# chaiyujin/sdfa-2019

Hardware: AMD Instinct MI355X
Metric: animation frames/s/node (10 s@16 kHz clips); max|Δdgrad| vs CPU ref (higher is better)
Workload: dtype f32

## Files before the change

include/sdfa_hip.h:

```cpp
#ifndef SDFA_HIP_H
#define SDFA_HIP_H

#include <stdint.h>

#ifdef __cplusplus
extern "C" {
#endif

#define SDFA_ABI_VERSION 5

#define SDFA_OK            0
#define SDFA_EINVAL       -1
#define SDFA_ESHORTCLIP   -2
#define SDFA_EHIP         -3
#define SDFA_ESTATE       -4
#define SDFA_ENOSPACE     -5

#define SDFA_HEAD_DGRAD    0
#define SDFA_HEAD_OFFSETS  1

#define SDFA_FEAT_FRAMES   64
#define SDFA_FEAT_MELS    128
#define SDFA_FEAT_CH        3
#define SDFA_Z_DIM        512
// ... 27 lines not shown
int         sdfa_model_finalize(sdfa_model *m, void *stream);
int         sdfa_model_head(const sdfa_model *m);
int64_t     sdfa_model_out_dim(const sdfa_model *m);
int64_t     sdfa_model_coef_dim(const sdfa_model *m);

#define SDFA_PREC_FP32 0
#define SDFA_PREC_BF16_ATTENTION 1
#define SDFA_PREC_BF16X3 2
#define SDFA_PREC_BF16 3
#define SDFA_PREC_BF16X3_ATTENTION 4
#define SDFA_PREC_BF16X6 5
int         sdfa_model_set_precision(sdfa_model *m, int mode);
int         sdfa_model_precision(const sdfa_model *m);

int         sdfa_model_autotune(sdfa_model *m, int64_t n_frames, void *d_workspace, int64_t workspace_bytes, void *stream);

int         sdfa_model_set_reserved_cus(sdfa_model *m, int k);

int64_t sdfa_workspace_bytes(const sdfa_model *m, int64_t max_frames);

#define SDFA_WS_STATUS_BYTES 256
#define SDFA_WS_STATUS_WORDS 4
#define SDFA_WS_TIME_LSTM_REPAIRS 0
int     sdfa_workspace_init(void *d_workspace, int64_t workspace_bytes, void *stream);
int     sdfa_workspace_status_async(const void *d_workspace, uint32_t *h_status, void *stream);
int64_t sdfa_workspace_status(const void *d_workspace, int word, void *stream);

int sdfa_encoder_forward(const sdfa_model *m, const float *d_audio_feat, int64_t n_frames,
                         float *d_z, float *d_align, void *d_workspace, int64_t workspace_bytes,
                         void *stream);

int sdfa_encoder_forward_shared(const sdfa_model *m, const float *d_audio_feat, int64_t n_frames,
                                const int32_t *d_frame_clip, const int64_t *d_frame_start, int hop,
                                float *d_z, float *d_align, void *d_workspace, int64_t workspace_bytes,
                                void *stream);

int sdfa_regress_forward(const sdfa_model *m, const float *d_z, const int64_t *d_speaker_id,
                         int64_t n_frames, float *d_coef, float *d_out, void *d_workspace,
                         int64_t workspace_bytes, void *stream);

int sdfa_regress_forward_multi(const sdfa_model *m, const float *d_z, const int64_t *d_speaker_id, int64_t n_frames,
                               float *d_coef, float *const *h_d_outs, int n_outs, void *d_workspace,
                               int64_t workspace_bytes, void *stream);

int sdfa_expand_coef(const sdfa_model *m, const float *d_coef, int64_t n_frames, float *d_out, void *d_workspace,
                     int64_t workspace_bytes, void *stream);
// ... 54 lines not shown
```

sdfa-2019_amd/csrc/api_core.cpp:

```cpp
#include "../../include/sdfa_stream.h"
#include "host.h"

#include <climits>
#include <cstdio>
#include <cstring>
#include <string>

static thread_local std::string g_err;

int sdfa_failv(int code, const char *fmt, va_list ap) {
    char buf[512];
    vsnprintf(buf, sizeof buf, fmt, ap);
    g_err = buf;
    return code;
}

int sdfa_fail(int code, const char *fmt, ...) {
    va_list ap;
    va_start(ap, fmt);
    sdfa_failv(code, fmt, ap);
    va_end(ap);
    return code;
}

thread_local int g_sdfa_mel_fft_radix4 = 0;
thread_local int g_sdfa_gather_plain_order = 0;
thread_local int g_sdfa_frontend_two_kernel = 0;
thread_local int g_sdfa_frontend_stream_block = 0;
thread_local int g_sdfa_frontend_stream_slots = 0;
thread_local int g_sdfa_frontend_stream_spin_max = 0;
thread_local int g_sdfa_frontend_stream_phases = 0;
thread_local int g_sdfa_frontend_t_major = 0;
extern thread_local int g_sdfa_gemm_variant;
thread_local int g_sdfa_freq_lstm_shape = 0;
thread_local int g_sdfa_pca_lds = 0;
thread_local int g_sdfa_pca_fp32 = 0;
thread_local int g_sdfa_conv_fp32 = 0;
thread_local int g_sdfa_time_lstm_split = 0;
thread_local int g_sdfa_time_lstm_fuse_x = 0;
thread_local int g_sdfa_time_lstm_handoff = 0;
thread_local int g_sdfa_time_lstm_timeout_us = 0;
thread_local int g_sdfa_share_gx0_off = 0;
thread_local int g_sdfa_encoder_dedup_off = 0;
thread_local int g_sdfa_share_hash_bits = 0;
thread_local int g_sdfa_freq_proj_tail = 0;
thread_local int g_sdfa_attn_unfused = 0;

extern "C" {

int sdfa_abi_version(void) { return SDFA_ABI_VERSION; }
int sdfa_stream_abi_version(void) { return SDFA_STREAM_ABI_VERSION; }
const char *sdfa_last_error(void) { return g_err.c_str(); }

int sdfa_debug_set_option(const char *name, int value) {
    struct Option { const char *name; int *var; int lo = INT_MIN, hi = INT_MAX; const char *accepts = nullptr; };
    thread_local const Option options[] = {
        {"attn_unfused", &g_sdfa_attn_unfused},
        {"share_gx0_off", &g_sdfa_share_gx0_off},
        {"encoder_dedup_off", &g_sdfa_encoder_dedup_off},
        {"share_hash_bits", &g_sdfa_share_hash_bits, 0, 32, "0 (the whole hash) or 1..32 low bits"},
        {"freq_proj_tail", &g_sdfa_freq_proj_tail, 0, 2, "0 (rule), 1 (never) or 2 (always)"},
        {"frontend_two_kernel", &g_sdfa_frontend_two_kernel},
        {"frontend_stream_phases", &g_sdfa_frontend_stream_phases},
        {"frontend_stream_spin_max", &g_sdfa_frontend_stream_spin_max, 0, INT_MAX, "0 (default) or a positive poll count"},
        {"frontend_stream_block", &g_sdfa_frontend_stream_block, 0, 256, "0 (default) or 1..256 frames"},
        {"frontend_stream_slots", &g_sdfa_frontend_stream_slots, 0, 256, "0 (default) or 1..256 workgroups per block"},
        {"gather_plain_order", &g_sdfa_gather_plain_order},
        {"mel_fft_radix4", &g_sdfa_mel_fft_radix4},
        {"frontend_t_major", &g_sdfa_frontend_t_major},
        {"time_lstm_timeout_us", &g_sdfa_time_lstm_timeout_us},
        {"time_lstm_handoff", &g_sdfa_time_lstm_handoff},
        {"time_lstm_split", &g_sdfa_time_lstm_split},
        {"time_lstm_fuse_x", &g_sdfa_time_lstm_fuse_x, 0, 3, "0 (rule), 1 (never), 2 or 3 (always, 32- / 64-frame tiles)"},
        {"gemm_variant", &g_sdfa_gemm_variant},
        {"freq_lstm_shape", &g_sdfa_freq_lstm_shape},
        {"pca_lds", &g_sdfa_pca_lds},
        {"conv_fp32", &g_sdfa_conv_fp32},
        {"pca_fp32", &g_sdfa_pca_fp32},
    };
    for (const Option &o : options)
        if (name && !strcmp(name, o.name)) {
            if (value < o.lo || value > o.hi) return sdfa_fail(SDFA_EINVAL, "%s: %s", o.name, o.accepts);
            *o.var = value;
            return SDFA_OK;
// ... 6 lines not shown
```

sdfa-2019_amd/csrc/api_forward.cpp:

```cpp
#include "common.h"
#include "host.h"
#include "kernels.h"
#include "model.h"

#include <algorithm>

extern thread_local int g_sdfa_gemm_variant, g_sdfa_freq_lstm_shape, g_sdfa_pca_lds, g_sdfa_pca_fp32, g_sdfa_conv_fp32, g_sdfa_share_gx0_off, g_sdfa_attn_unfused, g_sdfa_encoder_dedup_off,
    g_sdfa_freq_proj_tail, g_sdfa_share_hash_bits;

namespace {

constexpr int64_t CT_WORDS = 2048, CT_FLAGS = 16, ST_WORDS = SDFA_WS_STATUS_BYTES / 4;

struct Ws {
    int64_t P1, X3, HF, Z, GX, H0, H1, KP, QC, QP, ZK, SH, ZU, total;
    int64_t TRUNK, A0, A1, COEF;
    int64_t CT_FREQ, CT_PCA, CT_FLAG;
};

Ws layout(int64_t Nc, bool keep) {
    const int64_t Mc = 64 * Nc;
    Ws w{};
    int64_t o = 0;
    auto take = [&](int64_t n) { int64_t r = o; o += round_up(n, 64); return r; };
    take(ST_WORDS);
    if (keep) {
        w.P1 = take(2048 * Mc); w.X3 = take(2048 * Mc); w.HF = take((int64_t)HF_SLAB_ROWS * 4 * Mc); w.Z = take(256 * Mc);
        w.GX = take(2048 * Mc); w.H0 = take(512 * Mc); w.H1 = take(512 * Mc); w.KP = take(128 * Mc);
    } else {
        const int64_t A = take(2048 * Mc);
        const int64_t B = take(2048 * Mc);
// ... 124 lines not shown
    if (((uintptr_t)d_workspace | (uintptr_t)d_audio_feat | (uintptr_t)d_z | (uintptr_t)d_H | (uintptr_t)d_X1) & 15) return sdfa_fail(SDFA_EINVAL, "encoder_forward: pointers must be 16-byte aligned");
    if ((uintptr_t)d_align & 3) return sdfa_fail(SDFA_EINVAL, "encoder_forward: d_align must be 4-byte aligned");
    const int64_t cap = capacity(workspace_bytes, m->keep);
    if (cap < 128) return sdfa_fail(SDFA_ENOSPACE, "encoder_forward: workspace of %lld bytes holds no 128-frame chunk", (long long)workspace_bytes);
    hipStream_t s = (hipStream_t)stream;
    Prof pf{m, s};
    float *ws = (float *)d_workspace;
    for (int64_t f0 = 0; f0 < n_frames; f0 += cap) {
        const int64_t N = std::min(cap, n_frames - f0);
        const int64_t Nc = round_up(N, 128), Mc = 64 * Nc;
        const Ws w = layout(Nc, m->keep);
        ConvArgs ca{};
        ca.audio_feat = d_audio_feat + f0 * (64 * 128 * 3); ca.N = N; ca.Nc = Nc; ca.Mc = Mc;
        ca.w1 = m->w1; ca.b1 = m->b1; ca.s1 = m->s1; ca.t1 = m->t1; ca.P1 = ws + w.P1;
        ca.w2 = m->w2; ca.b2 = m->b2; ca.s2 = m->s2; ca.t2 = m->t2;
        ca.w3 = m->w3; ca.b3 = m->b3; ca.s3 = m->s3; ca.t3 = m->t3; ca.X3 = ws + w.X3;
        const bool table = d_frame_clip != nullptr;
        const bool share = table || (!m->keep && !g_sdfa_encoder_dedup_off);
        const int64_t *d_ulimit = nullptr;
        int32_t *col_to_u = nullptr;
        bool split_tail = false;
        int64_t fat_grid = 0;
        const int64_t *d_qfull = nullptr;
        if (share) {
            ShareArgs sa{};
            sa.N = N; sa.Nc = Nc; sa.Mc = Mc;
            sdfa_share_carve(sa, reinterpret_cast<int32_t *>(ws + w.SH));
            split_tail = !m->keep && stage_terms(m, STAGE_BODY) == 0 && g_sdfa_gemm_variant == 0 && Mc / 256 >= 512 && g_sdfa_freq_proj_tail != 1;
            if (split_tail) {
                fat_grid = sdfa_fat_grid(256, Mc, sdfa_cu_count(), m->reserved_cus.load());
                sa.fat_grid = (int)fat_grid; sa.tail_mode = g_sdfa_freq_proj_tail;
            }
            pf.begin("share_map");
            if (table) {
                sa.frame_clip = d_frame_clip + f0; sa.frame_start = d_frame_start + f0; sa.hop = hop;
                sa.t_lo = 6; sa.t_hi = 58;
                HIP_TRY(sdfa_launch_share_map(sa, s));
            } else {
                sa.feat = ca.audio_feat;
                sa.hash = reinterpret_cast<uint64_t *>(ws + w.HF);
                sa.group_slots = sdfa_share_group_slots(N);
                sa.group_key = sa.hash + Mc; sa.group_first = reinterpret_cast<uint32_t *>(sa.group_key + sa.group_slots);
                sa.hash_bits = g_sdfa_share_hash_bits;
                HIP_TRY(sdfa_launch_share_map_content(sa, s));
            }
            pf.end();
            d_ulimit = sa.counts + 1; d_qfull = sa.counts + 2; col_to_u = sa.col_to_u;
            ca.col_src = sa.col_src; ca.col_limit = d_ulimit;
        }
        const int conv_terms = g_sdfa_conv_fp32 ? 0 : stage_terms(m, STAGE_BODY);
        if (m->keep && conv_terms) {
            pf.begin("conv1"); HIP_TRY(sdfa_launch_conv1(ca, s)); pf.end();
            ca.wb = m->cv_wb; ca.terms = conv_terms;
            pf.begin("conv23"); HIP_TRY(sdfa_launch_conv123(ca, s)); pf.end();
        } else if (m->keep) {
            pf.begin("conv1"); HIP_TRY(sdfa_launch_conv1(ca, s)); pf.end();
            pf.begin("conv23"); HIP_TRY(sdfa_launch_conv23(ca, s)); pf.end();
        } else {
            ca.wb = m->cv_wb; ca.terms = conv_terms;
            pf.begin("conv23"); HIP_TRY(sdfa_launch_conv123(ca, s)); pf.end();
        }

        const int fl_terms = stage_terms(m, STAGE_BODY);
        FreqLstmArgs fa{ws + w.X3, m->fl_w, m->fl_b, ws + w.HF, Mc, d_ulimit, m->fl_wb, fl_terms, reinterpret_cast<int *>(ws + w.CT_FREQ),
                        g_sdfa_freq_lstm_shape ? g_sdfa_freq_lstm_shape : (fl_terms ? 0 : m->freq_shape.load()), m->reserved_cus.load()};
        pf.begin("freq_lstm"); HIP_TRY(sdfa_launch_freq_lstm(fa, s)); pf.end();

        GemmArgs g = sdfa_gemm_k4(m->fp_w, 256, ws + w.HF, Mc, ws + w.Z, Mc, 8192);
        g.bias = m->fp_b; g.q_tile_major = 1; g.q_slab_rows = HF_SLAB_ROWS;
        g.terms = stage_terms(m, STAGE_BODY);
        g.reserve_cus = m->reserved_cus.load();
        if (share) { g.D = ws + w.ZU; g.q_limit = split_tail ? d_qfull : d_ulimit; }
        pf.begin("freq_proj");
        HIP_TRY(sdfa_launch_gemm(g, s));
        if (split_tail) {
            GemmTailArgs gt{m->fp_w, ws + w.HF, m->fp_b, ws + w.ZU, Mc, HF_SLAB_ROWS, d_qfull, d_ulimit, (int)fat_grid - 1};
            HIP_TRY(sdfa_launch_gemm_tail(gt, s));
        }
        pf.end();
        const bool share_gx0 = share && !m->keep && stage_terms(m, STAGE_BODY) == 0 && !g_sdfa_share_gx0_off;
        if (share && !share_gx0) {
            pf.begin("share_expand"); HIP_TRY(sdfa_launch_expand_cols(ws + w.ZU, col_to_u, ws + w.Z, 64, Mc, s)); pf.end();
        }

        const float *xin = share_gx0 ? ws + w.ZU : ws + w.Z;
        float *hout[2] = {ws + w.H0, ws + w.H1};
        const char *gxn[2] = {"gx0", "gx1"}, *lsn[2] = {"lstm0", "lstm1"};
        for (int l = 0; l < 2; ++l) {
            const bool mapped = share_gx0 && l == 0;
            float *gx = mapped ? ws + w.HF : ws + w.GX;
            GemmArgs gi = sdfa_gemm_k4(m->gx_w[l], 2048, xin, Mc, gx, Mc, l == 0 ? 256 : 512);
            gi.terms = stage_terms(m, STAGE_BODY);
            gi.reserve_cus = m->reserved_cus.load();
            if (mapped) gi.q_limit = d_ulimit;
            TimeLstmArgs ta{gx, m->tl_w[l], hout[l], Nc, Mc, m->tl_wb[l], stage_terms(m, STAGE_BODY),
                            reinterpret_cast<unsigned *>(ws + w.CT_FLAG), CT_WORDS - CT_FLAGS, m->tl_w16[l],
                            reinterpret_cast<unsigned *>(ws), m->reserved_cus.load(), mapped ? col_to_u : nullptr};
            if (l == 1 && !m->keep) { ta.X = xin; ta.Wxh = m->tl_wxh1; }
            pf.begin(gxn[l]);
            if (!sdfa_time_lstm_fuses_x(ta)) HIP_TRY(sdfa_launch_gemm(gi, s));
            pf.end();
            pf.begin(lsn[l]); HIP_TRY(sdfa_launch_time_lstm(ta, s)); pf.end();
            xin = hout[l];
            if (d_X1) break;
        }
        if (d_X1) {
            HIP_TRY(sdfa_launch_tap(ws + w.H0, 3, N, Nc, d_X1 + f0 * (64 * 512), s));
            continue;
        }
        const int at_terms = stage_terms(m, STAGE_ATTENTION);
        const bool key_fused = g_sdfa_attn_unfused != 1;
        pf.begin("attn_proj");
        GemmArgs gk = sdfa_gemm_k4(m->kp_w, 128, ws + w.H1, Mc, ws + w.KP, Mc, 512);
        gk.terms = at_terms;
        if (!key_fused) HIP_TRY(sdfa_launch_gemm(gk, s));
        GemmArgs gc = sdfa_gemm_k4(m->qc_w, 512, ws + w.H1 + 31 * Nc * 4, Mc, ws + w.QC, Nc, 1536);
        gc.seg_k = 512; gc.seg_col = Nc; gc.terms = at_terms;
        HIP_TRY(sdfa_launch_gemm(gc, s));
        GemmArgs gq = sdfa_gemm_k4(m->qp_w, 128, ws + w.QC, Nc, ws + w.QP, Nc, 512);
        gq.terms = at_terms;
        HIP_TRY(sdfa_launch_gemm(gq, s));
        const bool tail_fused = key_fused && (at_terms == 0 || at_terms == 6) && g_sdfa_attn_unfused != 2 && sdfa_attn_fuses_tail(Nc, m->reserved_cus.load());
        if (key_fused) {
// ... 253 lines not shown
```

sdfa-2019_amd/csrc/gemm.hip:

```cpp
#include "common.h"
#include "kernels.h"

extern thread_local int g_sdfa_gemm_variant;

namespace {

constexpr int TP = 128, TQ = 128, KQ = 8;

template <int OUT_MODE, int ACT, bool BIAS_P, bool BIAS_Q, bool COND>
__device__ __forceinline__ void store_tile(const GemmArgs &a, const f32x16 &acc, int64_t p_tile, int64_t q, int h) {
    float bq = 0.f;
    if (BIAS_Q) bq = (q < a.Qreal) ? a.bias[q] : 0.f;
    int spk = 0;
    if (COND) { spk = (int)a.cond_idx[q < a.Qreal ? q : 0]; spk = spk < 0 ? 0 : (spk > 7 ? 7 : spk); }
#pragma unroll
    for (int g = 0; g < 4; ++g) {
        const int64_t p = p_tile + 8 * g + 4 * h;
        float v[4] = {acc[4 * g + 0], acc[4 * g + 1], acc[4 * g + 2], acc[4 * g + 3]};
        if (BIAS_P) {
            float4 b = ld4(a.bias + p);
            v[0] += b.x; v[1] += b.y; v[2] += b.z; v[3] += b.w;
        }
        if (COND) {
            float4 c = ld4(a.cond_w + (p / 4 * 8 + spk) * 4);
// ... 846 lines not shown
            __builtin_amdgcn_sched_barrier(0);                                                                   \
        }                                                                                                        \
        if (fetching) FAT_DMA_NEXT()                                                                             \
        mfma_block<4, 4>(acc, fa1, fb1);                                                                         \
        mfma_block<4, 4>(acc, fa2, fb2);                                                                         \
        __builtin_amdgcn_sched_barrier(0);                                                                       \
         \
        __builtin_amdgcn_s_waitcnt(0x0070);                                                                      \
        __syncthreads();                                      \
        {               \
            const float4 *sp = SP((BUF) ^ 1), *sq = SQ((BUF) ^ 1);                                               \
            FAT_READ(sp, sq, 0, fa0, fb0)                                                                        \
            FAT_READ(sp, sq, 1, fa1, fb1)                                                                        \
            FAT_READ(sp, sq, 2, fa2, fb2)                                                                        \
            FAT_READ(sp, sq, 3, FREE_A, FREE_B)                                                                  \
            mfma_block<4, 4>(acc, LAST_A, LAST_B);                                                               \
            _Pragma("unroll") for (int m = 0; m < 8; ++m) {                                                      \
                __builtin_amdgcn_sched_group_barrier(0x100, 4, 0);                                               \
                __builtin_amdgcn_sched_group_barrier(0x008, 8, 0);                                               \
            }                                                                                                    \
        }                                                                                                        \
        __builtin_amdgcn_sched_barrier(0);                                                                       \
    }
    for (;;) {
        for (int st = 0; st < nstage; st += 2) {
            FAT_STAGE(0, fa3, fb3, fa4, fb4)
            FAT_STAGE(1, fa4, fb4, fa3, fb3)
        }
        {
            const int64_t p0 = (int64_t)t.tp * BT, q0 = (int64_t)t.tq * BT;
            char *dbase = reinterpret_cast<char *>(a.D) + (((p0 >> 2) + wp * 32) * a.ldd + q0 + wq * 128) * 16;
            const unsigned dlane = (unsigned)((h * a.ldd + l31) * 16);
#pragma unroll
            for (int i = 0; i < 4; ++i) {
                float4 b[4];
                if (BIAS_P) {
#pragma unroll
                    for (int g = 0; g < 4; ++g) b[g] = ld4(a.bias + p0 + wp * 128 + i * 32 + 8 * g + 4 * h);
                }
#pragma unroll
                for (int j = 0; j < 4; ++j) {
#pragma unroll
                    for (int g = 0; g < 4; ++g) {
                        float v[4] = {acc[i][j][4 * g + 0], acc[i][j][4 * g + 1], acc[i][j][4 * g + 2], acc[i][j][4 * g + 3]};
                        if (BIAS_P) { v[0] += b[g].x; v[1] += b[g].y; v[2] += b[g].z; v[3] += b[g].w; }
#pragma unroll
                        for (int e = 0; e < 4; ++e) {
                            if (ACT == ACT_LRELU) v[e] = lrelu02(v[e]);
                            if (ACT == ACT_TANH) v[e] = tanhf_acc(v[e]);
                        }
                        *reinterpret_cast<float4 *>(dbase + ((int64_t)(i * 8 + 2 * g) * a.ldd + j * 32) * 16 + dlane) = make_float4(v[0], v[1], v[2], v[3]);
                    }
#pragma unroll
                    for (int r = 0; r < 16; ++r) acc[i][j][r] = 0.f;
                }
            }
        }
        advance(t);
        if (!live(t)) break;
    }
#undef FAT_STAGE
#undef FAT_Q
#undef FAT_DMA_ROWS
#undef FAT_DMA_NEXT
#undef FAT_READ
}

template <int OUT_MODE, int ACT, bool BIAS_P, bool BIAS_Q, bool COND>
hipError_t launch_fat(const GemmArgs &a, hipStream_t s) {
    const size_t lds = 2 * 2 * KQ * 256 * sizeof(float4);
    hipError_t e = hipFuncSetAttribute(reinterpret_cast<const void *>(gemm_fat_kernel<OUT_MODE, ACT, BIAS_P, BIAS_Q, COND>),
                                       hipFuncAttributeMaxDynamicSharedMemorySize, (int)lds);
    if (e != hipSuccess) return e;
    const int64_t cus = sdfa_cu_count();
    const int64_t ntiles = (a.Ppad / 256) * (a.Qpad / 256);
    const int64_t wgs = std::max<int64_t>(1, cus - a.reserve_cus);
    hipLaunchKernelGGL((gemm_fat_kernel<OUT_MODE, ACT, BIAS_P, BIAS_Q, COND>), dim3((unsigned)std::min(ntiles, wgs)), dim3(256), lds, s, a);
    return hipGetLastError();
}

}

thread_local int g_sdfa_gemm_variant = 0;

template <int OUT_MODE, int ACT, bool BIAS_P, bool BIAS_Q, bool COND>
hipError_t launch_any(const GemmArgs &a, hipStream_t s) {
    const int variant = (g_sdfa_gemm_variant == 2 || g_sdfa_gemm_variant == 6 || g_sdfa_gemm_variant == 10 || g_sdfa_gemm_variant == 11) ? 0 : g_sdfa_gemm_variant;
    const bool big_fills_half = variant == 12 || (a.Ppad / 256) * (a.Qpad / 256) * 2 >= sdfa_cu_count();
    if (a.terms == 6)
// ... 1 lines not shown
                                                                                                           : launch_bf16x6<OUT_MODE, ACT, BIAS_P, BIAS_Q, COND>(a, s);
    if (a.terms) {
        const bool big = a.Ppad % 256 == 0 && a.Qpad % 256 == 0 && variant != 7 && big_fills_half;
        if (a.terms == 1) return big ? launch_bf16_big<OUT_MODE, ACT, BIAS_P, BIAS_Q, COND, 1>(a, s) : launch_bf16<OUT_MODE, ACT, BIAS_P, BIAS_Q, COND, 1>(a, s);
        return big ? launch_bf16_big<OUT_MODE, ACT, BIAS_P, BIAS_Q, COND, 3>(a, s) : launch_bf16<OUT_MODE, ACT, BIAS_P, BIAS_Q, COND, 3>(a, s);
    }
    if (variant == 4 && !a.q_tile_major) return launch_bf16<OUT_MODE, ACT, BIAS_P, BIAS_Q, COND, 3>(a, s);
    {
        const bool fits = a.Ppad % 256 == 0 && a.Qpad % 256 == 0 && a.seg_k == a.K && a.K % 64 == 0 && OUT_MODE == OUT_K4 && !BIAS_Q && !COND &&
                          a.Pstore == a.Ppad && a.ldd * 16 * 2 < (int64_t)1 << 32 &&
                          (int64_t)(a.K / 4) * a.ldp * 16 < 0x7fffffff && (int64_t)(a.K / 4) * (a.q_tile_major ? 128 : a.ldq) * 16 < 0x7fffffff;
        const int64_t ntiles = (a.Ppad / 256) * (a.Qpad / 256);
        if constexpr (OUT_MODE == OUT_K4 && !BIAS_Q && !COND) {
            if (fits && (variant == 8 || (variant == 0 && ntiles >= 512)))
                return launch_fat<OUT_MODE, ACT, BIAS_P, BIAS_Q, COND>(a, s);
        }
    }
    const bool big_fills = (a.Ppad / 256) * (a.Qpad / 256) >= 256;
    if ((variant == 5 || (a.q_tile_major && ((variant == 0 && big_fills) || variant == 9))) && a.Ppad % 256 == 0 && a.Qpad % 256 == 0)
        return launch_big<OUT_MODE, ACT, BIAS_P, BIAS_Q, COND>(a, s);
    return launch<OUT_MODE, ACT, BIAS_P, BIAS_Q, COND>(a, s);
}

hipError_t sdfa_launch_gemm(const GemmArgs &a, hipStream_t s) {
    if (a.K % 32 || a.seg_k % 32 || a.Ppad % TP || a.Qpad % TQ || a.K % a.seg_k) return hipErrorInvalidValue;
    const bool bp = a.bias && !a.bias_on_q, bq = a.bias && a.bias_on_q, cond = a.cond_w != nullptr;
    if (a.out_mode == OUT_ROW) {
        if (bq && a.act == ACT_NONE && !cond) return launch_any<OUT_ROW, ACT_NONE, false, true, false>(a, s);
        return hipErrorInvalidValue;
    }
    if (bq) return hipErrorInvalidValue;
    if (cond) {
        if (a.act == ACT_LRELU && bp) return launch_any<OUT_K4, ACT_LRELU, true, false, true>(a, s);
        return hipErrorInvalidValue;
    }
    if (a.act == ACT_NONE) return bp ? launch_any<OUT_K4, ACT_NONE, true, false, false>(a, s)
                                     : launch_any<OUT_K4, ACT_NONE, false, false, false>(a, s);
    if (a.act == ACT_TANH && bp) return launch_any<OUT_K4, ACT_TANH, true, false, false>(a, s);
    if (a.act == ACT_LRELU && bp) return launch_any<OUT_K4, ACT_LRELU, true, false, false>(a, s);
    return hipErrorInvalidValue;
}
```

sdfa-2019_amd/csrc/kernels.h:

```cpp
#pragma once
#include <hip/hip_runtime.h>
#include <stdint.h>

enum { ACT_NONE = 0, ACT_LRELU = 1, ACT_TANH = 2 };

constexpr int HF_SLAB_ROWS = 2048;
enum { OUT_K4 = 0, OUT_ROW = 1 };
constexpr int SDFA_MAX_DESTS = 8;

struct GemmArgs {
    const float *P;
    const float *Q;
    float *D;
    const float *bias;
    const float *cond_w;
    const int64_t *cond_idx;
    int64_t ldp, ldq, ldd;
    int64_t Ppad, Qpad;
    int64_t Pstore;
    int64_t Qreal;
    int K;
    int seg_k;
    int64_t seg_col;
    int act, out_mode, bias_on_q;
    int terms;
    int q_tile_major;
    int q_slab_rows;
    const int64_t *q_limit;
    int col_group, col_stride, col_off;
    float *D_extra[SDFA_MAX_DESTS - 1];
    int n_extra;
    int reserve_cus;
};
hipError_t sdfa_launch_gemm(const GemmArgs &a, hipStream_t s);
inline GemmArgs sdfa_gemm_k4(const float *P, int64_t rows, const float *Q, int64_t ldq, float *D, int64_t cols, int K) {
    GemmArgs g{};
    g.P = P; g.Q = Q; g.D = D;
    g.ldp = rows; g.Ppad = rows; g.Pstore = rows;
    g.ldq = ldq; g.ldd = cols; g.Qpad = cols; g.Qreal = cols;
    g.K = K; g.seg_k = K; g.act = ACT_NONE; g.out_mode = OUT_K4;
    return g;
}

struct PcaArgs {
    const float *coef;
    const float *basis_s, *basis_r;
    const float *mean_s, *mean_r;
    float *out;
    int64_t N, Nc, out_dim, ld_s, ld_r, cols_s, cols_r;
    float *out_extra[SDFA_MAX_DESTS - 1];
    int n_extra;
    int reserve_cus;
    const void *basis_b;
    int terms;
};
hipError_t sdfa_launch_pca_dgrad(const PcaArgs &a, hipStream_t s);
hipError_t sdfa_launch_pca_dgrad_res(const PcaArgs &a, int *queue, hipStream_t s);

struct FrontendConsts {
    const float *hamm;
    const float2 *twiddle;
    const int *mel_bin0;
    const float *mel_w8;
    int win, hop, sliding, nbins_used, nnz;
};
// ... 106 lines not shown
hipError_t sdfa_launch_k4_to_rows(const float *src, int64_t ld, int64_t N, int F, int f0, int nf, float *dst,
                                  int64_t dst_ld, hipStream_t s);
hipError_t sdfa_launch_tap(const float *src, int what, int64_t N, int64_t Nc, float *dst, hipStream_t s);

struct ShareArgs {
    const int32_t *frame_clip;
    const int64_t *frame_start;
    int hop;
    int t_lo, t_hi;
    int frame_major;
    int64_t N, Nc, Mc;
    int32_t *prev, *shift;
    int32_t *owner, *flag, *uid;
    int32_t *tile_sum;
    int32_t *col_src;
    int32_t *col_to_u;
    int64_t *counts;
    const float *feat;
    uint64_t *hash;
    uint64_t *group_key;
    uint32_t *group_first;
    int64_t group_slots;
    int hash_bits;
    int fat_grid;
    int tail_mode;
};
inline int64_t sdfa_share_table_words(int64_t Nc) { return 16 + 2 * Nc + 5 * (64 * Nc) + (64 * Nc) / 1024 + 1; }
inline int64_t sdfa_share_group_slots(int64_t N) { int64_t s = 1024; while (s < 2 * 64 * N) s <<= 1; return s; }
inline void sdfa_share_carve(ShareArgs &a, int32_t *base) {
    a.counts = reinterpret_cast<int64_t *>(base);
    a.prev = base + 16; a.shift = a.prev + a.Nc;
    a.owner = a.shift + a.Nc; a.flag = a.owner + a.Mc; a.uid = a.flag + a.Mc;
    a.col_src = a.uid + a.Mc; a.col_to_u = a.col_src + a.Mc; a.tile_sum = a.col_to_u + a.Mc;
}
hipError_t sdfa_launch_share_map(const ShareArgs &a, hipStream_t s);
hipError_t sdfa_launch_share_map_content(const ShareArgs &a, hipStream_t s);
hipError_t sdfa_launch_share_prev(const ShareArgs &a, hipStream_t s);
hipError_t sdfa_launch_expand_cols(const float *Zu, const int32_t *col_to_u, float *Z, int nquads, int64_t Mc, hipStream_t s);

struct GemmTailArgs {
    const float *P, *Q, *bias;
    float *D;
    int64_t ldd;
    int q_slab_rows;
    const int64_t *q_lo, *q_hi;
    int max_tiles;
// ... 75 lines not shown
```

sdfa-2019_amd/csrc/share.hip:

```cpp
#include "common.h"
#include "kernels.h"

namespace {


__global__ void share_prev_kernel(ShareArgs a) {
    const int64_t n = (int64_t)blockIdx.x * blockDim.x + threadIdx.x;
    if (n >= a.Nc) return;
    int prev = -1, shift = 0;
    if (n < a.N) {
        const int clip = a.frame_clip[n];
        const int64_t s = a.frame_start[n];
        for (int back = 1; back <= 64 && n - back >= 0; ++back) {
            const int64_t q = n - back;
            if (a.frame_clip[q] != clip) break;
            const int64_t diff = s - a.frame_start[q];
            if (diff <= 0) break;
            if (diff > (int64_t)(a.t_hi - a.t_lo) * a.hop) break;
            if (diff % a.hop == 0) { prev = (int)q; shift = (int)(diff / a.hop); break; }
        }
    }
    a.prev[n] = prev;
    a.shift[n] = shift;
}
// ... 118 lines not shown
}

__global__ __launch_bounds__(1024) void share_scan_tiles_kernel(ShareArgs a) {
    __shared__ int part[1024];
    const int64_t i = (int64_t)blockIdx.x * 1024 + threadIdx.x;
    const int f = i < a.Mc ? a.flag[i] : 0;
    const int inc = block_inclusive_scan_1024(f, part);
    if (i < a.Mc) a.uid[i] = inc - f;
    if (threadIdx.x == 1023) a.tile_sum[blockIdx.x] = inc;
}

constexpr int TAIL_NUM = 3, TAIL_DEN = 4;
__global__ __launch_bounds__(1024) void share_scan_sums_kernel(ShareArgs a, int ntiles) {
    __shared__ int part[1024];
    int carry = 0;
    for (int base = 0; base < ntiles; base += 1024) {
        const int t = base + threadIdx.x;
        const int v = t < ntiles ? a.tile_sum[t] : 0;
        const int inc = block_inclusive_scan_1024(v, part);
        if (t < ntiles) a.tile_sum[t] = carry + inc - v;
        carry += part[1023];
        __syncthreads();
    }
    if (threadIdx.x == 0) {
        const int64_t mu = carry, pad = (mu + 255) / 256 * 256;
        a.counts[0] = mu;
        a.counts[1] = pad;
        int64_t q_full = pad;
        if (a.fat_grid > 0 && a.tail_mode != 1) {
            const int64_t T = pad / 256, G = a.fat_grid, r = T % G;
            if (a.tail_mode == 2 || r * TAIL_DEN <= G * TAIL_NUM) q_full = (T - r) * 256;
        }
        a.counts[2] = q_full;
    }
}

__global__ __launch_bounds__(1024) void share_scan_fix_kernel(ShareArgs a) {
    const int64_t i = (int64_t)blockIdx.x * 1024 + threadIdx.x;
    const int64_t mu = a.counts[0], pad = a.counts[1];
    if (i < a.Mc) {
        const int u = a.uid[i] + a.tile_sum[blockIdx.x];
        a.uid[i] = u;
        int64_t n;
        int t;
        col_of(a, i, n, t);
        if (a.flag[i]) a.col_src[u] = (int)(n * 64 + t);
// ... 56 lines not shown
```

sdfa-2019_amd/sdfa_amd/engine.py:

```python
import ctypes as C

import numpy as np
import torch

from . import _lib
from ._lib import lib, check
from .weights import fold_state_dict, head_of, check_strict

FPS = 60
TS_DELTA_MS = 100
FEAT_SHAPE = (64, 128, 3)


def frame_geometry(sr):
    win, hop = int(0.064 * sr), int(0.008 * sr)
    return win, hop, hop * 63 + win


def frame_index(n_samples, sr, fps=FPS, ts_delta=TS_DELTA_MS):
    win, hop, _ = frame_geometry(sr)
    n = check(lib.sdfa_frame_index(int(n_samples), int(sr), int(fps), win, hop, int(ts_delta), None, None, 0))
    starts = np.empty(n, np.int64)
    ts = np.empty(n, np.int32)
    check(lib.sdfa_frame_index(int(n_samples), int(sr), int(fps), win, hop, int(ts_delta),
# ... 132 lines not shown
        self.precision = precision

    def __del__(self):
        m, self._m = getattr(self, "_m", None), None
        if m:
            lib.sdfa_model_destroy(m)

    def workspace(self, n_frames):
        need = check(lib.sdfa_workspace_bytes(self._m, min(int(n_frames), self.max_frames)))
        if self._ws is None or self._ws.numel() < need:
            if self._ws is not None:
                self.check_pending(block=True)
                carried = self.time_lstm_repairs()
                self._repairs_carried = carried
            self._ws = None
            self._ws = torch.empty(need, dtype=torch.uint8, device=self.device)
            check(lib.sdfa_workspace_init(_ptr(self._ws), self._ws.numel(), _stream()))
        return self._ws

    def time_lstm_repairs(self):
        if self._ws is None:
            return self._repairs_carried
        return self._repairs_carried + int(check(lib.sdfa_workspace_status(_ptr(self._ws), 0, _stream())))

    def _status_async(self, stream_ptr=None):
        if self._ws is None:
            return
        slot = self._status_free.pop() if self._status_free else torch.zeros(4, dtype=torch.int32, pin_memory=True)
        check(lib.sdfa_workspace_status_async(_ptr(self._ws), _ptr(slot), stream_ptr if stream_ptr is not None else _stream()))
        ev = torch.cuda.Event()
        ev.record(torch.cuda.current_stream(self.device))
        self._status_reads.append((slot, ev))

    def autotune(self, n_frames=None):
        n = min(int(n_frames or self.max_frames), self.max_frames)
        ws = self.workspace(n)
        self.freq_lstm_form = int(check(lib.sdfa_model_autotune(self._m, n, _ptr(ws), ws.numel(), _stream())))
        self._autotune_pending = False
        return self.freq_lstm_form

    def encoder(self, audio_feat, want_align=True, frame_clip=None, frame_start=None, hop=None):
        assert audio_feat.is_cuda and audio_feat.dtype == torch.float32 and tuple(audio_feat.shape[1:]) == FEAT_SHAPE
        audio_feat = audio_feat.contiguous()
        n = audio_feat.shape[0]
        z = torch.empty((n, 512), dtype=torch.float32, device=self.device)
        align = torch.empty((n, 64), dtype=torch.float32, device=self.device) if want_align else None
# ... 345 lines not shown
```

Baseline: 150,000.

## Chain freq projection GEMM and gx0 GEMM in one persistent kernel with tile stamps

Fuses the freq_proj GEMM and the first-layer gx0 input GEMM into one persistent kernel. The first phase publishes per-column-tile completion stamps, and the second phase pulls work from an atomic queue, starting a tile as soon as its input tile is ready. Tiles whose stamps do not appear within a timeout are deferred to a second repair launch. The goal is to remove the kernel boundary and tail idle time between the two GEMMs and to drop the separate gx0 launch. In exchange it adds spin-waiting, atomics and fence costs, and the output now goes to a different workspace buffer (Z and GX instead of ZU and HF).

```diff
diff --git a/include/sdfa_hip.h b/include/sdfa_hip.h
--- a/include/sdfa_hip.h
+++ b/include/sdfa_hip.h
@@ -73,6 +73,7 @@
 #define SDFA_WS_STATUS_BYTES 256
 #define SDFA_WS_STATUS_WORDS 4
 #define SDFA_WS_TIME_LSTM_REPAIRS 0
+#define SDFA_WS_PROJ_CHAIN_DEFERRALS 1
 int     sdfa_workspace_init(void *d_workspace, int64_t workspace_bytes, void *stream);
 int     sdfa_workspace_status_async(const void *d_workspace, uint32_t *h_status, void *stream);
 int64_t sdfa_workspace_status(const void *d_workspace, int word, void *stream);
diff --git a/sdfa-2019_amd/csrc/api_core.cpp b/sdfa-2019_amd/csrc/api_core.cpp
--- a/sdfa-2019_amd/csrc/api_core.cpp
+++ b/sdfa-2019_amd/csrc/api_core.cpp
@@ -44,6 +44,8 @@
 thread_local int g_sdfa_encoder_dedup_off = 0;
 thread_local int g_sdfa_share_hash_bits = 0;
 thread_local int g_sdfa_freq_proj_tail = 0;
+thread_local int g_sdfa_proj_chain = 0;
+thread_local int g_sdfa_proj_chain_wait_us = 0;
 thread_local int g_sdfa_attn_unfused = 0;
 
 extern "C" {
@@ -60,6 +62,8 @@
         {"encoder_dedup_off", &g_sdfa_encoder_dedup_off},
         {"share_hash_bits", &g_sdfa_share_hash_bits, 0, 32, "0 (the whole hash) or 1..32 low bits"},
         {"freq_proj_tail", &g_sdfa_freq_proj_tail, 0, 2, "0 (rule), 1 (never) or 2 (always)"},
+        {"proj_chain", &g_sdfa_proj_chain, 0, 2, "0 (rule), 1 (off) or 2 (always)"},
+        {"proj_chain_wait_us", &g_sdfa_proj_chain_wait_us, -1, INT_MAX, "0 (default), -1 (no waiting) or a positive number of microseconds"},
         {"frontend_two_kernel", &g_sdfa_frontend_two_kernel},
         {"frontend_stream_phases", &g_sdfa_frontend_stream_phases},
         {"frontend_stream_spin_max", &g_sdfa_frontend_stream_spin_max, 0, INT_MAX, "0 (default) or a positive poll count"},
diff --git a/sdfa-2019_amd/csrc/api_forward.cpp b/sdfa-2019_amd/csrc/api_forward.cpp
--- a/sdfa-2019_amd/csrc/api_forward.cpp
+++ b/sdfa-2019_amd/csrc/api_forward.cpp
@@ -6,7 +6,7 @@
 #include <algorithm>
 
 extern thread_local int g_sdfa_gemm_variant, g_sdfa_freq_lstm_shape, g_sdfa_pca_lds, g_sdfa_pca_fp32, g_sdfa_conv_fp32, g_sdfa_share_gx0_off, g_sdfa_attn_unfused, g_sdfa_encoder_dedup_off,
-    g_sdfa_freq_proj_tail, g_sdfa_share_hash_bits;
+    g_sdfa_freq_proj_tail, g_sdfa_share_hash_bits, g_sdfa_proj_chain, g_sdfa_proj_chain_wait_us;
 
 namespace {
 
@@ -177,11 +177,20 @@
         bool split_tail = false;
         int64_t fat_grid = 0;
         const int64_t *d_qfull = nullptr;
+        const bool chain = share && !m->keep && stage_terms(m, STAGE_BODY) == 0 && g_sdfa_gemm_variant == 0 && Mc / 256 >= 512 && Mc < ((int64_t)1 << 21) &&
+                           !g_sdfa_share_gx0_off && g_sdfa_freq_proj_tail == 0 && g_sdfa_proj_chain != 1;
+        GemmChainArgs ch{};
         if (share) {
             ShareArgs sa{};
             sa.N = N; sa.Nc = Nc; sa.Mc = Mc;
             sdfa_share_carve(sa, reinterpret_cast<int32_t *>(ws + w.SH));
-            split_tail = !m->keep && stage_terms(m, STAGE_BODY) == 0 && g_sdfa_gemm_variant == 0 && Mc / 256 >= 512 && g_sdfa_freq_proj_tail != 1;
+            split_tail = !chain && !m->keep && stage_terms(m, STAGE_BODY) == 0 && g_sdfa_gemm_variant == 0 && Mc / 256 >= 512 && g_sdfa_freq_proj_tail != 1;
+            if (chain) {
+                ch.ctl = reinterpret_cast<unsigned *>(sa.counts) + 9;
+                ch.stamp = reinterpret_cast<unsigned *>(sa.prev);
+                ch.deferred = reinterpret_cast<unsigned *>(sa.flag);
+                sa.chain_ctl = ch.ctl; sa.chain_stamp = ch.stamp; sa.chain_stamps = Mc / 256;
+            }
             if (split_tail) {
                 fat_grid = sdfa_fat_grid(256, Mc, sdfa_cu_count(), m->reserved_cus.load());
                 sa.fat_grid = (int)fat_grid; sa.tail_mode = g_sdfa_freq_proj_tail;
@@ -225,9 +234,18 @@
         g.bias = m->fp_b; g.q_tile_major = 1; g.q_slab_rows = HF_SLAB_ROWS;
         g.terms = stage_terms(m, STAGE_BODY);
         g.reserve_cus = m->reserved_cus.load();
-        if (share) { g.D = ws + w.ZU; g.q_limit = split_tail ? d_qfull : d_ulimit; }
+        float *zu = chain ? ws + w.Z : ws + w.ZU, *gx0 = chain ? ws + w.GX : ws + w.HF;
+        if (share) { g.D = zu; g.q_limit = split_tail ? d_qfull : d_ulimit; }
         pf.begin("freq_proj");
-        HIP_TRY(sdfa_launch_gemm(g, s));
+        if (chain) {
+            ch.A = g;
+            ch.B = sdfa_gemm_k4(m->gx_w[0], 2048, zu, Mc, gx0, Mc, 256);
+            ch.B.q_limit = d_ulimit; ch.B.reserve_cus = g.reserve_cus;
+            ch.status = reinterpret_cast<unsigned *>(ws) + SDFA_WS_PROJ_CHAIN_DEFERRALS;
+            const int us = g_sdfa_proj_chain_wait_us;
+            ch.wait_ticks = us < 0 ? 0u : (unsigned)std::min<int64_t>((int64_t)(us ? us : 20000) * 100, 0xffffffffll);
+            HIP_TRY(sdfa_launch_gemm_chain(ch, s));
+        } else HIP_TRY(sdfa_launch_gemm(g, s));
         if (split_tail) {
             GemmTailArgs gt{m->fp_w, ws + w.HF, m->fp_b, ws + w.ZU, Mc, HF_SLAB_ROWS, d_qfull, d_ulimit, (int)fat_grid - 1};
             HIP_TRY(sdfa_launch_gemm_tail(gt, s));
@@ -238,12 +256,12 @@
             pf.begin("share_expand"); HIP_TRY(sdfa_launch_expand_cols(ws + w.ZU, col_to_u, ws + w.Z, 64, Mc, s)); pf.end();
         }
 
-        const float *xin = share_gx0 ? ws + w.ZU : ws + w.Z;
+        const float *xin = share_gx0 ? zu : ws + w.Z;
         float *hout[2] = {ws + w.H0, ws + w.H1};
         const char *gxn[2] = {"gx0", "gx1"}, *lsn[2] = {"lstm0", "lstm1"};
         for (int l = 0; l < 2; ++l) {
             const bool mapped = share_gx0 && l == 0;
-            float *gx = mapped ? ws + w.HF : ws + w.GX;
+            float *gx = mapped ? gx0 : ws + w.GX;
             GemmArgs gi = sdfa_gemm_k4(m->gx_w[l], 2048, xin, Mc, gx, Mc, l == 0 ? 256 : 512);
             gi.terms = stage_terms(m, STAGE_BODY);
             gi.reserve_cus = m->reserved_cus.load();
@@ -253,7 +271,7 @@
                             reinterpret_cast<unsigned *>(ws), m->reserved_cus.load(), mapped ? col_to_u : nullptr};
             if (l == 1 && !m->keep) { ta.X = xin; ta.Wxh = m->tl_wxh1; }
             pf.begin(gxn[l]);
-            if (!sdfa_time_lstm_fuses_x(ta)) HIP_TRY(sdfa_launch_gemm(gi, s));
+            if (!(mapped && chain) && !sdfa_time_lstm_fuses_x(ta)) HIP_TRY(sdfa_launch_gemm(gi, s));
             pf.end();
             pf.begin(lsn[l]); HIP_TRY(sdfa_launch_time_lstm(ta, s)); pf.end();
             xin = hout[l];
diff --git a/sdfa-2019_amd/csrc/gemm.hip b/sdfa-2019_amd/csrc/gemm.hip
--- a/sdfa-2019_amd/csrc/gemm.hip
+++ b/sdfa-2019_amd/csrc/gemm.hip
@@ -892,49 +892,229 @@
         }                                                                                                        \
         __builtin_amdgcn_sched_barrier(0);                                                                       \
     }
+#define FAT_EPILOGUE()                                                                                                  \
+    {                                                                                                                   \
+        const int64_t p0 = (int64_t)t.tp * BT, q0 = (int64_t)t.tq * BT;                                                 \
+        char *dbase = reinterpret_cast<char *>(a.D) + (((p0 >> 2) + wp * 32) * a.ldd + q0 + wq * 128) * 16;             \
+        const unsigned dlane = (unsigned)((h * a.ldd + l31) * 16);                                                      \
+        _Pragma("unroll")                                                                                               \
+        for (int i = 0; i < 4; ++i) {                                                                                   \
+            float4 b[4];                                                                                                \
+            if (BIAS_P) {                                                                                               \
+                _Pragma("unroll")                                                                                       \
+                for (int g = 0; g < 4; ++g) b[g] = ld4(a.bias + p0 + wp * 128 + i * 32 + 8 * g + 4 * h);                \
+            }                                                                                                           \
+            _Pragma("unroll")                                                                                           \
+            for (int j = 0; j < 4; ++j) {                                                                               \
+                _Pragma("unroll")                                                                                       \
+                for (int g = 0; g < 4; ++g) {                                                                           \
+                    float v[4] = {acc[i][j][4 * g + 0], acc[i][j][4 * g + 1], acc[i][j][4 * g + 2], acc[i][j][4 * g + 3]};\
+                    if (BIAS_P) { v[0] += b[g].x; v[1] += b[g].y; v[2] += b[g].z; v[3] += b[g].w; }                     \
+                    _Pragma("unroll")                                                                                   \
+                    for (int e = 0; e < 4; ++e) {                                                                       \
+                        if (ACT == ACT_LRELU) v[e] = lrelu02(v[e]);                                                     \
+                        if (ACT == ACT_TANH) v[e] = tanhf_acc(v[e]);                                                    \
+                    }                                                                                                   \
+                    *reinterpret_cast<float4 *>(dbase + ((int64_t)(i * 8 + 2 * g) * a.ldd + j * 32) * 16 + dlane) = make_float4(v[0], v[1], v[2], v[3]);\
+                }                                                                                                       \
+                _Pragma("unroll")                                                                                       \
+                for (int r = 0; r < 16; ++r) acc[i][j][r] = 0.f;                                                        \
+            }                                                                                                           \
+        }                                                                                                               \
+    }
     for (;;) {
         for (int st = 0; st < nstage; st += 2) {
             FAT_STAGE(0, fa3, fb3, fa4, fb4)
             FAT_STAGE(1, fa4, fb4, fa3, fb3)
         }
-        {
-            const int64_t p0 = (int64_t)t.tp * BT, q0 = (int64_t)t.tq * BT;
-            char *dbase = reinterpret_cast<char *>(a.D) + (((p0 >> 2) + wp * 32) * a.ldd + q0 + wq * 128) * 16;
-            const unsigned dlane = (unsigned)((h * a.ldd + l31) * 16);
-#pragma unroll
-            for (int i = 0; i < 4; ++i) {
-                float4 b[4];
-                if (BIAS_P) {
-#pragma unroll
-                    for (int g = 0; g < 4; ++g) b[g] = ld4(a.bias + p0 + wp * 128 + i * 32 + 8 * g + 4 * h);
-                }
-#pragma unroll
-                for (int j = 0; j < 4; ++j) {
-#pragma unroll
-                    for (int g = 0; g < 4; ++g) {
-                        float v[4] = {acc[i][j][4 * g + 0], acc[i][j][4 * g + 1], acc[i][j][4 * g + 2], acc[i][j][4 * g + 3]};
-                        if (BIAS_P) { v[0] += b[g].x; v[1] += b[g].y; v[2] += b[g].z; v[3] += b[g].w; }
-#pragma unroll
-                        for (int e = 0; e < 4; ++e) {
-                            if (ACT == ACT_LRELU) v[e] = lrelu02(v[e]);
-                            if (ACT == ACT_TANH) v[e] = tanhf_acc(v[e]);
-                        }
-                        *reinterpret_cast<float4 *>(dbase + ((int64_t)(i * 8 + 2 * g) * a.ldd + j * 32) * 16 + dlane) = make_float4(v[0], v[1], v[2], v[3]);
-                    }
-#pragma unroll
-                    for (int r = 0; r < 16; ++r) acc[i][j][r] = 0.f;
-                }
-            }
-        }
+        FAT_EPILOGUE()
         advance(t);
         if (!live(t)) break;
     }
+}
+
+enum { CH_NEXT = 0, CH_DONE = 1, CH_DEFER = 2, CH_REPAIR = 3 };
+enum { CHV_GO = 0, CHV_ACQUIRE = 1, CHV_END = 2 };
+
+__device__ __forceinline__ unsigned chain_wait(const unsigned *ps, unsigned ticks) {
+    if (ticks == 0) return 0;
+    unsigned spins = 0;
+    unsigned long long t0 = 0;
+    for (;;) {
+        const unsigned v = __hip_atomic_load(ps, __ATOMIC_RELAXED, __HIP_MEMORY_SCOPE_AGENT);
+        if (v) return v;
+        if ((++spins & 63u) == 0u) {
+            const unsigned long long now = __builtin_amdgcn_s_memrealtime();
+            if (t0 == 0) t0 = now;
+            else if (now - t0 > (unsigned long long)ticks) return 0;
+        }
+        __builtin_amdgcn_s_sleep(8);
+    }
+}
+
+template <bool BIAS_P, bool QUEUE>
+__device__ __forceinline__ void fat_chain_phase(const GemmArgs &a, const GemmChainArgs &c, unsigned &seen, unsigned *s_q) {
+    constexpr int BT = 256, ACT = ACT_NONE;
+    extern __shared__ float4 sFat[];
+    const int tid = threadIdx.x, lane = tid & 63;
+    const int wave = __builtin_amdgcn_readfirstlane(tid >> 6);
+    const int wp = wave >> 1, wq = wave & 1, l31 = lane & 31, h = lane >> 5;
+    const int64_t ntp = a.Ppad / BT;
+    const int64_t q_end = a.q_limit ? std::min<int64_t>(*a.q_limit, a.Qpad) : a.Qpad;
+
+    const float4 *__restrict__ P = reinterpret_cast<const float4 *>(a.P);
+    const float4 *__restrict__ Q = reinterpret_cast<const float4 *>(a.Q);
+    const int nstage = a.K / 32;
+    auto SP = [&](int buf) { return sFat + (size_t)buf * 2 * KQ * BT; };
+    auto SQ = [&](int buf) { return sFat + (size_t)buf * 2 * KQ * BT + KQ * BT; };
+    const int64_t qrow = a.q_tile_major ? 128 : a.ldq;
+    const unsigned voff = (unsigned)lane * 16;
+    struct Tile { int tp, tq; };
+    const int g_tp = (int)(gridDim.x % ntp), g_tq = (int)(gridDim.x / ntp), ntp_i = (int)ntp;
+    const Tile END{0, 1 << 22};
+    auto live = [&](const Tile &x) { return (int64_t)x.tq * BT < q_end; };
+
+    const unsigned n_tiles = (unsigned)(ntp * (q_end / BT));
+    const unsigned n_items = QUEUE && c.repair ? std::min(__hip_atomic_load(c.ctl + CH_DEFER, __ATOMIC_RELAXED, __HIP_MEMORY_SCOPE_AGENT), n_tiles) : n_tiles;
+    const bool ahead = QUEUE && !c.repair && nstage >= 6;
+    unsigned r_tk = 0, r_s = 0;
+    bool have_ahead = false;
+    auto from_ticket = [&](unsigned tk) { return Tile{(int)(tk % (unsigned)ntp_i), (int)(tk / (unsigned)ntp_i)}; };
+    auto resolve = [&]() -> Tile {
+        unsigned tk = r_tk, s = r_s;
+        const bool have = have_ahead;
+        have_ahead = false;
+        if (have) {
+            if (tk >= n_items) return END;
+            if (s != 0 && s <= seen) return from_ticket(tk);
+        }
+        __syncthreads();
+        if (tid == 0) {
+            unsigned v = CHV_GO, sn = seen;
+            bool fresh = !have;
+            for (;;) {
+                if (fresh) {
+                    tk = __hip_atomic_fetch_add(c.ctl + (c.repair ? CH_REPAIR : CH_NEXT), 1u, __ATOMIC_RELAXED, __HIP_MEMORY_SCOPE_AGENT);
+                    s = (!c.repair && tk < n_items) ? __hip_atomic_load(c.stamp + tk / (unsigned)ntp_i, __ATOMIC_RELAXED, __HIP_MEMORY_SCOPE_AGENT) : 0u;
+                }
+                fresh = true;
+                if (tk >= n_items) { v = CHV_END; break; }
+                if (c.repair) {
+                    tk = c.deferred[tk];
+                    if (tk >= n_tiles) v = CHV_END;
+                    break;
+                }
+                if (s == 0) s = chain_wait(c.stamp + tk / (unsigned)ntp_i, c.wait_ticks);
+                if (s == 0) {
+                    const unsigned d = __hip_atomic_fetch_add(c.ctl + CH_DEFER, 1u, __ATOMIC_RELAXED, __HIP_MEMORY_SCOPE_AGENT);
+                    if (d < n_tiles) c.deferred[d] = tk;
+                    if (c.status) __hip_atomic_fetch_add(c.status, 1u, __ATOMIC_RELAXED, __HIP_MEMORY_SCOPE_AGENT);
+                    continue;
+                }
+                if (s > seen) {
+                    const unsigned x = __hip_atomic_load(c.ctl + CH_DONE, __ATOMIC_RELAXED, __HIP_MEMORY_SCOPE_AGENT);
+                    sn = x > s ? x : s;
+                    v = CHV_ACQUIRE;
+                }
+                break;
+            }
+            s_q[4] = tk; s_q[5] = v; s_q[6] = sn;
+        }
+        __syncthreads();
+        tk = s_q[4];
+        const unsigned v = s_q[5];
+        if (v == CHV_ACQUIRE) {
+            seen = s_q[6];
+            if (wave == 0) {
+                __builtin_amdgcn_fence(__ATOMIC_ACQUIRE, "agent");
+                __builtin_amdgcn_s_waitcnt(0x0070);
+            }
+            __syncthreads();
+        }
+        return v == CHV_END ? END : from_ticket(tk);
+    };
+    auto advance = [&](Tile &x) {
+        if constexpr (QUEUE) x = resolve();
+        else { x.tp += g_tp; x.tq += g_tq; if (x.tp >= ntp_i) { x.tp -= ntp_i; ++x.tq; } }
+    };
+    const __amdgpu_buffer_rsrc_t prs = __builtin_amdgcn_make_buffer_rsrc(const_cast<float4 *>(P), 0, 0x7fffffff, 0x00020000);
+    auto p_off = [&](const Tile &x) { return (unsigned)(((int64_t)x.tp * BT + wave * 64) * 16); };
+    auto q_rsrc = [&](const Tile &x) {
+        const int64_t q0 = (int64_t)x.tq * BT;
+        const float4 *b = a.q_tile_major ? Q + ((q0 >> 7) + (wave >> 1)) * (int64_t)a.q_slab_rows * 128 + (wave & 1) * 64 : Q + q0 + wave * 64;
+        return __builtin_amdgcn_make_buffer_rsrc(const_cast<float4 *>(b), 0, 0x7fffffff, 0x00020000);
+    };
+
+    Tile t{(int)(blockIdx.x % ntp), (int)(blockIdx.x / ntp)};
+    if constexpr (QUEUE) t = resolve();
+    if (!live(t)) return;
+    Tile tf = t;
+    unsigned po = p_off(tf), qo = 0;
+    __amdgpu_buffer_rsrc_t qrs = q_rsrc(tf);
+    const unsigned p_row = (unsigned)(a.ldp * 16), q_row = (unsigned)(qrow * 16);
+    int fetch_left = nstage;
+    bool fetching = true;
+    f32x16 acc[4][4];
+#pragma unroll
+    for (int i = 0; i < 4; ++i)
+#pragma unroll
+        for (int j = 0; j < 4; ++j)
+#pragma unroll
+            for (int r = 0; r < 16; ++r) acc[i][j][r] = 0.f;
+
+    float4 fa0[4], fb0[4], fa1[4], fb1[4], fa2[4], fb2[4], fa3[4], fb3[4], fa4[4], fb4[4];
+    FAT_DMA_ROWS(0, 0, KQ)
+    FAT_DMA_NEXT()
+    __builtin_amdgcn_s_waitcnt(0x0070);
+    __syncthreads();
+    FAT_READ(SP(0), SQ(0), 0, fa0, fb0)
+    FAT_READ(SP(0), SQ(0), 1, fa1, fb1)
+    FAT_READ(SP(0), SQ(0), 2, fa2, fb2)
+    FAT_READ(SP(0), SQ(0), 3, fa3, fb3)
+    unsigned pf_tk = 0, pf_s = 0;
+    for (;;) {
+        for (int st = 0; st < nstage; st += 2) {
+            if (ahead && st == 0 && tid == 0)
+                pf_tk = __hip_atomic_fetch_add(c.ctl + CH_NEXT, 1u, __ATOMIC_RELAXED, __HIP_MEMORY_SCOPE_AGENT);
+            if (ahead && st == nstage - 2) {
+                r_tk = __builtin_amdgcn_readfirstlane(s_q[0]); r_s = __builtin_amdgcn_readfirstlane(s_q[1]);
+                have_ahead = true;
+            }
+            FAT_STAGE(0, fa3, fb3, fa4, fb4)
+            if (ahead && st == 0 && tid == 0)
+                pf_s = pf_tk < n_items ? __hip_atomic_load(c.stamp + pf_tk / (unsigned)ntp_i, __ATOMIC_RELAXED, __HIP_MEMORY_SCOPE_AGENT) : 0u;
+            FAT_STAGE(1, fa4, fb4, fa3, fb3)
+            if (ahead && st == 0 && tid == 0) { s_q[0] = pf_tk; s_q[1] = pf_s; }
+        }
+        FAT_EPILOGUE()
+        if (!QUEUE) {
+            __builtin_amdgcn_s_waitcnt(0x0070);
+            __syncthreads();
+            if (tid == 0) {
+                __builtin_amdgcn_fence(__ATOMIC_RELEASE, "agent");
+                __builtin_amdgcn_s_waitcnt(0x0070);
+                const unsigned n = __hip_atomic_fetch_add(c.ctl + CH_DONE, 1u, __ATOMIC_RELAXED, __HIP_MEMORY_SCOPE_AGENT);
+                __hip_atomic_store(c.stamp + t.tq, n + 1u, __ATOMIC_RELAXED, __HIP_MEMORY_SCOPE_AGENT);
+            }
+        }
+        if (!fetching) break;
+        t = tf;
+    }
+}
+
+__global__ __launch_bounds__(256, 1) void gemm_fat_chain_kernel(GemmChainArgs c) {
+    extern __shared__ float4 sFat[];
+    unsigned *s_q = reinterpret_cast<unsigned *>(sFat + 2 * 2 * KQ * 256);
+    unsigned seen = 0;
+    if (!c.repair) fat_chain_phase<true, false>(c.A, c, seen, s_q);
+    fat_chain_phase<false, true>(c.B, c, seen, s_q);
+}
 #undef FAT_STAGE
 #undef FAT_Q
 #undef FAT_DMA_ROWS
 #undef FAT_DMA_NEXT
 #undef FAT_READ
-}
+#undef FAT_EPILOGUE
 
 template <int OUT_MODE, int ACT, bool BIAS_P, bool BIAS_Q, bool COND>
 hipError_t launch_fat(const GemmArgs &a, hipStream_t s) {
@@ -982,6 +1162,29 @@
     return launch<OUT_MODE, ACT, BIAS_P, BIAS_Q, COND>(a, s);
 }
 
+hipError_t sdfa_launch_gemm_chain(const GemmChainArgs &c, hipStream_t s) {
+    auto fits = [](const GemmArgs &a) {
+        return a.Ppad % 256 == 0 && a.Qpad % 256 == 0 && a.seg_k == a.K && a.K % 64 == 0 && a.out_mode == OUT_K4 && !a.bias_on_q && !a.cond_w &&
+               a.act == ACT_NONE && a.terms == 0 && a.Pstore == a.Ppad && a.ldp == a.Ppad && a.ldd >= a.Qpad && a.ldd * 16 * 2 < (int64_t)1 << 32 &&
+               (int64_t)(a.K / 4) * a.ldp * 16 < 0x7fffffff && (int64_t)(a.K / 4) * (a.q_tile_major ? 128 : a.ldq) * 16 < 0x7fffffff;
+    };
+    const GemmArgs &A = c.A, &B = c.B;
+    if (!fits(A) || !fits(B) || A.Ppad != 256 || !A.bias || B.bias || B.Q != A.D || B.ldq != A.ldd || B.q_tile_major || A.Qpad != B.Qpad ||
+        A.q_limit != B.q_limit || !c.ctl || !c.stamp || !c.deferred || c.repair)
+        return hipErrorInvalidValue;
+    if (A.q_tile_major && A.q_slab_rows < A.K / 4) return hipErrorInvalidValue;
+    const size_t lds = 2 * 2 * KQ * 256 * sizeof(float4) + 64;
+    hipError_t e = hipFuncSetAttribute(reinterpret_cast<const void *>(gemm_fat_chain_kernel), hipFuncAttributeMaxDynamicSharedMemorySize, (int)lds);
+    if (e != hipSuccess) return e;
+    const int64_t wgs = std::max<int64_t>(1, sdfa_cu_count() - A.reserve_cus);
+    const unsigned grid = (unsigned)std::min(A.Qpad / 256, wgs);
+    hipLaunchKernelGGL(gemm_fat_chain_kernel, dim3(grid), dim3(256), lds, s, c);
+    GemmChainArgs r = c;
+    r.repair = 1;
+    hipLaunchKernelGGL(gemm_fat_chain_kernel, dim3(grid), dim3(256), lds, s, r);
+    return hipGetLastError();
+}
+
 hipError_t sdfa_launch_gemm(const GemmArgs &a, hipStream_t s) {
     if (a.K % 32 || a.seg_k % 32 || a.Ppad % TP || a.Qpad % TQ || a.K % a.seg_k) return hipErrorInvalidValue;
     const bool bp = a.bias && !a.bias_on_q, bq = a.bias && a.bias_on_q, cond = a.cond_w != nullptr;
diff --git a/sdfa-2019_amd/csrc/kernels.h b/sdfa-2019_amd/csrc/kernels.h
--- a/sdfa-2019_amd/csrc/kernels.h
+++ b/sdfa-2019_amd/csrc/kernels.h
@@ -41,6 +41,17 @@
     g.K = K; g.seg_k = K; g.act = ACT_NONE; g.out_mode = OUT_K4;
     return g;
 }
+
+struct GemmChainArgs {
+    GemmArgs A, B;
+    unsigned *ctl;
+    unsigned *stamp;
+    unsigned *deferred;
+    unsigned *status;
+    unsigned wait_ticks;
+    int repair;
+};
+hipError_t sdfa_launch_gemm_chain(const GemmChainArgs &c, hipStream_t s);
 
 struct PcaArgs {
     const float *coef;
@@ -193,6 +204,9 @@
     uint32_t *group_first;
     int64_t group_slots;
     int hash_bits;
+    unsigned *chain_ctl;
+    unsigned *chain_stamp;
+    int64_t chain_stamps;
     int fat_grid;
     int tail_mode;
 };
diff --git a/sdfa-2019_amd/csrc/share.hip b/sdfa-2019_amd/csrc/share.hip
--- a/sdfa-2019_amd/csrc/share.hip
+++ b/sdfa-2019_amd/csrc/share.hip
@@ -164,6 +164,10 @@
         carry += part[1023];
         __syncthreads();
     }
+    if (a.chain_ctl) {
+        if (threadIdx.x < 4) a.chain_ctl[threadIdx.x] = 0;
+        for (int64_t i = threadIdx.x; i < a.chain_stamps; i += 1024) a.chain_stamp[i] = 0;
+    }
     if (threadIdx.x == 0) {
         const int64_t mu = carry, pad = (mu + 255) / 256 * 256;
         a.counts[0] = mu;
diff --git a/sdfa-2019_amd/sdfa_amd/engine.py b/sdfa-2019_amd/sdfa_amd/engine.py
--- a/sdfa-2019_amd/sdfa_amd/engine.py
+++ b/sdfa-2019_amd/sdfa_amd/engine.py
@@ -178,6 +178,11 @@
         if self._ws is None:
             return self._repairs_carried
         return self._repairs_carried + int(check(lib.sdfa_workspace_status(_ptr(self._ws), 0, _stream())))
+
+    def proj_chain_deferrals(self):
+        if self._ws is None:
+            return 0
+        return int(check(lib.sdfa_workspace_status(_ptr(self._ws), 1, _stream())))
 
     def _status_async(self, stream_ptr=None):
         if self._ws is None:
```

After: 151,000 (median of 6 runs). No clear change (+0.6%).
